# jbejjani2022/InferBiomechanics

Measured on AMD Instinct MI355X. Metric: motion-windows/sec training (+ DDIM steps/sec), higher is better.
Workload: dtype bf16; 1 GPU; transformer_denoiser_T50_D300_B256_bf16 (BASELINE.json configs[2]); per_gpu_batch=256, global_batch=256, window=50, feat=300, optimizer=rmsprop, hipgraph=True, parallelism=dp1, grad_buckets=0, overlap_comm=False, loop_stream=trainer (HipTrainer.adopt_stream, as cli/train.py)

## Files before the change

__graft_entry__.py:

```python
import os
import subprocess
import sys

ROOT = os.path.dirname(os.path.abspath(__file__))
if ROOT not in sys.path:
    sys.path.insert(0, ROOT)


def build() -> None:
    csrc = os.path.join(ROOT, "inferbiomechanics_amd", "csrc")
    jobs = str(min(8, os.cpu_count() or 1))
    subprocess.run(["make", "-C", csrc, "-j", jobs, "ARCH=gfx950"], check=True)
    from inferbiomechanics_amd import hip
    lib = hip.lib()
    missing = [s for s in hip.declared_symbols() + hip.stitch_symbols() + hip.head_symbols() + hip.sde_symbols() + hip.cfg_symbols()
               + hip.ensemble_symbols() + hip.clip_decls() + hip.standardize_decls() + hip.sched_decls() + hip.decay_decls()
               if not hasattr(lib, s)]
    if missing:
        raise RuntimeError(f"libib_hip.so does not export: {missing}")
    import inferbiomechanics_amd


def smoke() -> None:
    import argparse

    import torch

    from inferbiomechanics_amd import hip
    from inferbiomechanics_amd.loss.DiffusionLossEvaluator import DiffusionLossEvaluator
    from inferbiomechanics_amd.loss.RegressionLossEvaluator import RegressionLossEvaluator
    from inferbiomechanics_amd.models.DiffusionDenoisers import DiffusionMLP
# ... 99 lines not shown
```

inferbiomechanics_amd/csrc/ffn_chain.h:

```cpp
#pragma once
#include "wave_prims.h"
#include <utility>

#ifdef IB_AB
extern long long* g_ffn_prof;
#endif

namespace {

constexpr int FF_ROWS = 64, FF_WAVES = 8, FF_THREADS = 512, FF_D = 512, FF_CHUNK = 512, FF_MAXCHUNK = 8;
constexpr int FF_NT = 4, FF_KB = 16;
constexpr int FF_RS = FF_D * 2 + 16;
constexpr int FF_BUF = FF_ROWS * FF_RS;
constexpr int64_t FF_WELEMS = (int64_t)FF_CHUNK * FF_D;

template <int CTRL>
__device__ __forceinline__ float ff_dpp_mov(float v) {
  return __builtin_bit_cast(float, __builtin_amdgcn_update_dpp(0, __builtin_bit_cast(int, v), CTRL, 0xF, 0xF, true));
}
template <int CTRL, int ROWMASK>
__device__ __forceinline__ float ff_dpp_bcast_add(float v) {
  return v + __builtin_bit_cast(float, __builtin_amdgcn_update_dpp(0, __builtin_bit_cast(int, v), CTRL, ROWMASK, 0xF, false));
}
__device__ __forceinline__ float ff_row_sum(float a) {
// ... 91 lines not shown

__device__ __forceinline__ int ff_fresh(int v) {
  asm volatile("" : "+v"(v));
  return v;
}
__device__ __forceinline__ int ff_colb() {
  const int t = ff_fresh(threadIdx.x);
  return (t & (FF_THREADS - 64)) | 4 * ((t >> 4) & 3);
}

template <class P>
using ff_karg_t = const __attribute__((address_space(4))) P;
template <class P>
__device__ __forceinline__ ff_karg_t<P>& ff_kargs() {
  return *(ff_karg_t<P>*)__builtin_amdgcn_kernarg_segment_ptr();
}


__device__ __forceinline__ void ff_ln_rows_fwd(unsigned char* img, bool back, int nrows, int wave_s, int lane,
                                               const float (&gm)[8], const float (&bt)[8], float eps, bf16_t* yg, bf16_t* sg,
                                               float* mean_g, float* rstd_g) {
  const float invH = 1.f / (float)FF_D;
  const int c8 = lane * 8;
  constexpr int G = 2;
#pragma unroll
  for (int j0 = 0; j0 < FF_ROWS / FF_WAVES; j0 += G) {
    if (!back && wave_s + FF_WAVES * j0 >= nrows) break;
    uint4 q[G];
    float v[G][8], s1[G], sq[G];
#pragma unroll
// ... 20 lines not shown
#pragma unroll
      for (int k = 0; k < 8; ++k) hv[k] = (v[gi][k] - mean) * rstd * gm[k] + bt[k];
      const uint4 hq = ff_pack8(hv);
      if (back) *reinterpret_cast<uint4*>(img + r * FF_RS + c8 * 2) = hq;
      if (r < nrows) {
        if (yg) *reinterpret_cast<uint4*>(yg + (int64_t)r * FF_D + c8) = hq;
        if (sg) {
          *reinterpret_cast<uint4*>(sg + (int64_t)r * FF_D + c8) = q[gi];
          if (lane == 0) { mean_g[r] = mean; rstd_g[r] = rstd; }
        }
      }
    }
  }
}

template <bool FROM_IMG>
__device__ __forceinline__ void ff_ln_rows_bwd(const bf16_t* dyg, const unsigned char* dyimg, const bf16_t* sg,
                                               const float* mean_g, const float* rstd_g, const float* gamma, int nrows,
                                               int wave_s, int lane, unsigned char* zimg, bf16_t* dzg, float (&dgam)[8],
                                               float (&dbet)[8]) {
  constexpr int NJ = FF_ROWS / FF_WAVES;
  const float invH = 1.f / (float)FF_D;
  const int c8 = lane * 8;
  uint4 qd[NJ], qs[NJ];
  float2 st[NJ];
#pragma unroll
  for (int j = 0; j < NJ; ++j) {
    const int r = wave_s + FF_WAVES * j, rc = min(r, nrows - 1);
    if constexpr (FROM_IMG) qd[j] = *reinterpret_cast<const uint4*>(dyimg + r * FF_RS + c8 * 2);
    else qd[j] = *reinterpret_cast<const uint4*>(dyg + (int64_t)rc * FF_D + c8);
    qs[j] = *reinterpret_cast<const uint4*>(sg + (int64_t)rc * FF_D + c8);
    st[j] = make_float2(mean_g[rc], rstd_g[rc]);
  }
  float gm[8];
  ff_load8f(gamma + c8, gm);
#pragma unroll
  for (int k = 0; k < 8; ++k) { dgam[k] = 0.f; dbet[k] = 0.f; }
  constexpr int G = 2;
#pragma unroll
  for (int j0 = 0; j0 < NJ; j0 += G) {
    float dxh[G][8], xh[G][8], sa[G], sb[G];
#pragma unroll
    for (int gi = 0; gi < G; ++gi) {
      const bool ok = wave_s + FF_WAVES * (j0 + gi) < nrows;
      float d[8], sv[8];
      ff_unpack8(qd[j0 + gi], d);
      ff_unpack8(qs[j0 + gi], sv);
      sa[gi] = 0.f; sb[gi] = 0.f;
#pragma unroll
      for (int k = 0; k < 8; ++k) {
// ... 9 lines not shown
#pragma unroll
    for (int gi = 0; gi < G; ++gi) { sa[gi] = ff_row_sum(sa[gi]); sb[gi] = ff_row_sum(sb[gi]); }
#pragma unroll
    for (int gi = 0; gi < G; ++gi) {
      const int r = wave_s + FF_WAVES * (j0 + gi);
      const float ma = sa[gi] * invH, mb = sb[gi] * invH;
      float dz[8];
#pragma unroll
      for (int k = 0; k < 8; ++k) dz[k] = st[j0 + gi].y * (dxh[gi][k] - ma - xh[gi][k] * mb);
      const uint4 zq = ff_pack8(dz);
      *reinterpret_cast<uint4*>(zimg + r * FF_RS + c8 * 2) = zq;
      if (r < nrows) *reinterpret_cast<uint4*>(dzg + (int64_t)r * FF_D + c8) = zq;
    }
  }
}
__device__ __forceinline__ void ff_colsum_put(float* cr, int wave, int lane, const float (&dgam)[8], const float (&dbet)[8]) {
  const int c8 = lane * 8;
  float* c0 = cr + (0 * FF_WAVES + wave) * FF_D + c8;
  float* c1 = cr + (1 * FF_WAVES + wave) * FF_D + c8;
  *reinterpret_cast<float4*>(c0) = make_float4(dgam[0], dgam[1], dgam[2], dgam[3]);
  *reinterpret_cast<float4*>(c0 + 4) = make_float4(dgam[4], dgam[5], dgam[6], dgam[7]);
  *reinterpret_cast<float4*>(c1) = make_float4(dbet[0], dbet[1], dbet[2], dbet[3]);
  *reinterpret_cast<float4*>(c1 + 4) = make_float4(dbet[4], dbet[5], dbet[6], dbet[7]);
}
__device__ __forceinline__ void ff_colsum_out(const float* cr, float* partial, int q0, int tid) {
  float s0 = 0.f, s1 = 0.f;
#pragma unroll
  for (int w = 0; w < FF_WAVES; ++w) {
    s0 += cr[(0 * FF_WAVES + w) * FF_D + tid];
    s1 += cr[(1 * FF_WAVES + w) * FF_D + tid];
// ... 85 lines not shown
```

inferbiomechanics_amd/csrc/ffn_chain.hip:

```cpp
#include "ffn_chain.h"
#include "../../include/ib_hip_head.h"
#include "head_jobs.h"

#ifdef IB_AB
long long* g_ffn_prof = nullptr;
#endif
namespace {

struct FfnFwdParams {
  const bf16_t* x1;
  const bf16_t* w1p; const bf16_t* w2p;
  const float* b1; const float* b2; const float* gamma; const float* beta;
  bf16_t* f1;
  bf16_t* s2;
  bf16_t* y;
  float* mean; float* rstd;
  uint2* mask;
  const bf16_t* attn; const bf16_t* wop; const float* bo; const float* gamma1; const float* beta1;
  bf16_t* s1; bf16_t* x1out; float* mean1; float* rstd1;
  const bf16_t* wqkvp; const float* bqkv; bf16_t* qkv;
  bf16_t* attn_next; float* lse_next;
  int M, P, FF, nchunk;
  float ln_eps;
  long long* prof;
};

template <bool OUT, bool QKV, bool ATT, bool INFER = false>
__global__ __launch_bounds__(FF_THREADS) void ffn_chain_fwd_kernel(FfnFwdParams) {
  ff_karg_t<FfnFwdParams>& p = ff_kargs<FfnFwdParams>();
  static_assert(!ATT || QKV, "the attention rides behind the QKV tail");
  static_assert(!INFER || (OUT && !ATT), "the frozen-weight form: attention epilogue, no attention tail");
  __shared__ __attribute__((aligned(16))) unsigned char smem[2 * FF_BUF];
  unsigned char* imgX = smem;
  unsigned char* imgH = smem + FF_BUF;
  const int tid = threadIdx.x, lane = tid & 63, wave = tid >> 6;
  const int wave_s = __builtin_amdgcn_readfirstlane(wave);
  const int g = lane >> 4, l16 = lane & 15;
  const int r0 = blockIdx.x * p.P;
  const int nrows = min(p.P, p.M - r0);
  const int colb = wave * 16 * FF_NT + 4 * g;
  const int c8 = lane * 8;
  IB_STAMP(p.prof, 64, 0, tid == 0);
  ff_panel_in(p.x1 + (int64_t)r0 * FF_D, imgX, nrows, tid);
  if constexpr (OUT) {
    ff_panel_in(p.attn + (int64_t)r0 * FF_D, imgH, nrows, tid);
    __syncthreads();
    f32x4_t acco[4][FF_NT];
    ff_zero(acco);
    float4 bo4[FF_NT];
    auto sideo = [&](auto, int kb) {
      if (kb == FF_KB - 1) {
#pragma unroll
        for (int u = 0; u < FF_NT; ++u) bo4[u] = *reinterpret_cast<const float4*>(p.bo + colb + 16 * u);
      }
    };
    ff_gemm<FF_RING_B>(p.wop, wave_s * FF_NT, imgH, lane_now(), acco, sideo);
    float gm1[8], bt1[8];
    ff_load8f(p.gamma1 + c8, gm1);
// ... 186 lines not shown
          *reinterpret_cast<bf16x4_t*>(imgH + (16 * it + l16) * FF_RS + (colb + 16 * dt) * 2) =
              ff_pack4(o[dt][0] * inv_l[it], o[dt][1] * inv_l[it], o[dt][2] * inv_l[it], o[dt][3] * inv_l[it]);
        }
      }
      __syncthreads();
      bf16_t* ag = p.attn_next + (int64_t)r0 * FF_D;
#pragma unroll
      for (int j = 0; j < 8; ++j) ff_out_piece(imgH, ag, FF_D, nrows, ff_fresh(tid + j * FF_THREADS));
    }
#pragma unroll
    for (int j = 0; j < 8; ++j) ff_out_piece(imgX, qg + 2 * FF_CHUNK, 3 * FF_D, nrows, ff_fresh(tid + j * FF_THREADS));
    IB_STAMP(p.prof, 64, 9 + 4 * p.nchunk, tid == 0);
  }
}


struct FfnPackDesc { const bf16_t* src; int64_t ld; int transpose; int pad; bf16_t* dst; };
constexpr int FF_MAXDESC = 96;
struct FfnPackParams { FfnPackDesc d[FF_MAXDESC]; int count; };
constexpr int FF_BLOCKS_PER_DESC = 32 * FF_KB;

constexpr int FF_MAXTR = 16, FF_MAXCAST = 2;
struct FfnPackExtra { TrMultiT<FF_MAXTR> tr; CastJob cast[FF_MAXCAST]; int pack_blocks, tr_blocks, cast_blocks[FF_MAXCAST]; };

__device__ __forceinline__ void ffn_pack_body(const FfnPackParams& p, bf16_t (*tile)[32][17], int first, int stride) {
  const int lane = threadIdx.x & 63, w = threadIdx.x >> 6;
  const int total = p.count * FF_BLOCKS_PER_DESC;
  for (int blk = first; blk < total; blk += stride) {
    const FfnPackDesc& d = p.d[blk / FF_BLOCKS_PER_DESC];
    const int local = blk % FF_BLOCKS_PER_DESC;
// ... 48 lines not shown
    }
    b -= x.cast_blocks[j];
  }
}

}

#ifdef IB_AB
extern "C" int ib_debug_set_ffn_prof(void* buf) { g_ffn_prof = reinterpret_cast<long long*>(buf); return IB_OK; }
#else
extern "C" int ib_debug_set_ffn_prof(void*) { return IB_E_UNSUPPORTED; }
#endif

extern "C" int ib_ffn_chain_supported(int64_t d, int64_t ffn) {
  return (d == FF_D && ffn > 0 && ffn % FF_CHUNK == 0 && ffn / FF_CHUNK <= FF_MAXCHUNK) ? 1 : 0;
}
extern "C" size_t ib_ffn_chain_packed_elems(int64_t d, int64_t ffn) {
  return ib_ffn_chain_supported(d, ffn) ? (size_t)((4 * (ffn / FF_CHUNK) + 8) * FF_WELEMS) : 0;
}
extern "C" int ib_ffn_chain_workgroups(int64_t M, int64_t d, int64_t ffn, int* rows_per_wg) {
  int P = 0, nc = 0;
  const int n = ffn_geometry(M, d, ffn, &P, &nc);
  if (rows_per_wg) *rows_per_wg = P;
  return n;
}
extern "C" size_t ib_ffn_chain_mask_bytes(int64_t M, int64_t d, int64_t ffn) {
  int P = 0, nc = 0;
  const int n = ffn_geometry(M, d, ffn, &P, &nc);
  return (size_t)n * nc * FF_THREADS * sizeof(uint2);
}
// ... 121 lines not shown
  const bf16_t* pk = reinterpret_cast<const bf16_t*>(packed);
  p.x1 = (const bf16_t*)x1; p.w1p = pk; p.w2p = pk + (int64_t)nc * FF_WELEMS;
  p.b1 = b1; p.b2 = b2; p.gamma = gamma; p.beta = beta;
  p.f1 = (bf16_t*)f1; p.s2 = (bf16_t*)s2; p.y = (bf16_t*)y; p.mean = mean; p.rstd = rstd; p.mask = (uint2*)mask;
  p.attn = (const bf16_t*)attn; p.wop = pk + (int64_t)4 * nc * FF_WELEMS; p.bo = bo; p.gamma1 = gamma1; p.beta1 = beta1;
  p.s1 = (bf16_t*)s1; p.x1out = (bf16_t*)x1_out; p.mean1 = mean1; p.rstd1 = rstd1;
  const bool tail = qkv_next != nullptr;
  if (tail && (!out || !packed_next || !bqkv_next || !ib_al16({packed_next, bqkv_next, qkv_next}))) return IB_E_ARG;
  if (att && (!tail || !lse_next || T <= 0 || P != T || !ib_al16({attn_next}))) return IB_E_ARG;
  p.wqkvp = tail ? reinterpret_cast<const bf16_t*>(packed_next) + (int64_t)(4 * nc + 2) * FF_WELEMS : nullptr;
  p.bqkv = bqkv_next; p.qkv = (bf16_t*)qkv_next;
  p.attn_next = (bf16_t*)attn_next; p.lse_next = lse_next;
  p.M = (int)M; p.P = P; p.FF = (int)ffn; p.nchunk = nc; p.ln_eps = ln_eps;
  p.prof = IB_AB_PROF(g_ffn_prof);
  IB_PATH(IB_PATH_FFN_CHAIN);
  if (att) hipLaunchKernelGGL((ffn_chain_fwd_kernel<true, true, true>), dim3(nwg), dim3(FF_THREADS), 0, ib_s(stream), p);
  else if (tail) hipLaunchKernelGGL((ffn_chain_fwd_kernel<true, true, false>), dim3(nwg), dim3(FF_THREADS), 0, ib_s(stream), p);
  else if (out) hipLaunchKernelGGL((ffn_chain_fwd_kernel<true, false, false>), dim3(nwg), dim3(FF_THREADS), 0, ib_s(stream), p);
  else hipLaunchKernelGGL((ffn_chain_fwd_kernel<false, false, false>), dim3(nwg), dim3(FF_THREADS), 0, ib_s(stream), p);
  IB_CHECK_LAUNCH();
  return IB_OK;
}
}

extern "C" int ib_ffn_chain_fwd(const void* x1, const void* packed, const float* b1, const float* b2, const float* gamma,
                                const float* beta, void* f1, void* s2, void* y, float* mean, float* rstd, void* mask,
                                const void* attn, const float* bo, const float* gamma1, const float* beta1, void* s1,
                                void* x1_out, float* mean1, float* rstd1, const void* packed_next, const float* bqkv_next,
                                void* qkv_next, int64_t M, int64_t d, int64_t ffn, float ln_eps, ib_stream_t stream) {
  return ffn_chain_fwd_launch(x1, packed, b1, b2, gamma, beta, f1, s2, y, mean, rstd, mask, attn, bo, gamma1, beta1, s1, x1_out,
                              mean1, rstd1, packed_next, bqkv_next, qkv_next, nullptr, nullptr, 0, M, d, ffn, ln_eps, stream);
}
extern "C" int ib_ffn_chain_fwd_infer(const void* x, const void* packed, const float* b1, const float* b2, const float* gamma,
                                      const float* beta, void* y, const void* attn, const float* bo, const float* gamma1,
// ... 35 lines not shown
```

inferbiomechanics_amd/csrc/ffn_chain_bwd.hip:

```cpp
#include "ffn_chain.h"

namespace {

struct FfnBwdParams {
  const bf16_t* dy;
  const bf16_t* s2;
  const float* mean; const float* rstd; const float* gamma;
  const bf16_t* w2tp; const bf16_t* w1tp;
  const uint2* mask;
  bf16_t* ds2;
  bf16_t* dz1;
  bf16_t* dx1;
  float* partial;
  const bf16_t* s1; const float* mean1; const float* rstd1; const float* gamma1; const bf16_t* wotp;
  bf16_t* ds1;
  bf16_t* dattn;
  const bf16_t* wqkvtp; const bf16_t* dqkv_next; const bf16_t* ds1_next;
  const bf16_t* qkv; const float* lse; bf16_t* dqkv; bf16_t* dx; const bf16_t* wqkvtp_own;
  int M, P, FF, nchunk;
  long long* prof;
};

__device__ __forceinline__ void ff_qkv_dgrad(const bf16_t* addend, const bf16_t* dq, const bf16_t* wqkvtp, unsigned char* imgZ,
                                             unsigned char* imgD, int nrows, int tid, int wave_s, int l16, int colb) {
  ff_panel_in(addend, imgZ, nrows, tid);
  ff_panel_in(dq, imgD, nrows, tid, 3 * FF_D);
  __syncthreads();
  f32x4_t accd[4][FF_NT];
  ff_zero(accd);
  for (int c = 0; c < 3; ++c) {
    uint4 n0, n1, n2, n3, n4, n5, n6, n7;
    n0 = n1 = n2 = n3 = n4 = n5 = n6 = n7 = make_uint4(0u, 0u, 0u, 0u);
    const bf16_t* dqn = dq + min(c + 1, 2) * FF_CHUNK;
    auto piece = [&](int j) {
      const int idx = FF_TIDV + j * FF_THREADS;
      return *reinterpret_cast<const uint4*>(reinterpret_cast<const unsigned char*>(dqn + (int64_t)min(idx >> 6, nrows - 1) * (3 * FF_D)) + (idx & 63) * 16);
    };
    auto sided = [&](auto kbc, int) {
      constexpr int kb = decltype(kbc)::value;
      if constexpr (kb == 0) n0 = piece(0);
// ... 17 lines not shown
    }
  }
#pragma unroll
  for (int u = 0; u < FF_NT; ++u) {
#pragma unroll
    for (int mt = 0; mt < 4; ++mt) {
      bf16x4_t* slot = reinterpret_cast<bf16x4_t*>(imgZ + (16 * mt + l16) * FF_RS + (colb + 16 * u) * 2);
      const bf16x4_t av = *slot;
      *slot = ff_pack4(accd[mt][u][0] + (float)av[0], accd[mt][u][1] + (float)av[1], accd[mt][u][2] + (float)av[2],
                       accd[mt][u][3] + (float)av[3]);
    }
  }
  __syncthreads();
}

template <bool OUT, bool QKVH, bool ATT>
__global__ __launch_bounds__(FF_THREADS) void ffn_chain_bwd_kernel(FfnBwdParams) {
  ff_karg_t<FfnBwdParams>& p = ff_kargs<FfnBwdParams>();
  static_assert(!ATT || OUT, "the attention backward rides behind the out-projection's dgrad");
  __shared__ float attL[ATT ? FF_WAVES : 1][64], attD[ATT ? FF_WAVES : 1][64];
  __shared__ __attribute__((aligned(16))) unsigned char smem[2 * FF_BUF];
  unsigned char* imgZ = smem;
  unsigned char* imgD = smem + FF_BUF;
  static_assert(2 * FF_WAVES * FF_D * 4 <= FF_BUF, "dgamma / dbeta exchange must fit an image");
  const int tid = threadIdx.x, lane = tid & 63, wave = tid >> 6;
  const int wave_s = __builtin_amdgcn_readfirstlane(wave);
  const int g = lane >> 4, l16 = lane & 15;
  const int r0 = blockIdx.x * p.P;
  const int nrows = min(p.P, p.M - r0);
  IB_STAMP(p.prof, 64, 0, tid == 0);
  if constexpr (QKVH) {
    ff_qkv_dgrad(p.ds1_next + (int64_t)r0 * FF_D, p.dqkv_next + (int64_t)r0 * (3 * FF_D), p.wqkvtp, imgZ, imgD, nrows, tid,
                 wave_s, l16, ff_colb());
  }
  {
    float dgam[8], dbet[8];
    ff_ln_rows_bwd<QKVH>(p.dy + (int64_t)r0 * FF_D, imgZ, p.s2 + (int64_t)r0 * FF_D, p.mean + r0, p.rstd + r0, p.gamma, nrows,
                         wave_s, lane, imgZ, p.ds2 + (int64_t)r0 * FF_D, dgam, dbet);
    ff_colsum_put(reinterpret_cast<float*>(imgD), wave, lane, dgam, dbet);
  }
  __syncthreads();
  ff_colsum_out(reinterpret_cast<const float*>(imgD), p.partial, 0, tid);
  __syncthreads();
  IB_STAMP(p.prof, 64, 1, tid == 0);

  f32x4_t accx[4][FF_NT];
  ff_zero(accx);
  for (int c = 0; c < p.nchunk; ++c) {
    f32x4_t acca[4][FF_NT];
    ff_zero(acca);
    uint2 mk = make_uint2(0u, 0u);
    auto sideA = [&](auto, int kb) {
      if (kb == FF_KB - 1) mk = p.mask[((int64_t)blockIdx.x * p.nchunk + c) * FF_THREADS + FF_TIDV];
// ... 253 lines not shown
      for (int u = 0; u < FF_NT; ++u) {
#pragma unroll
        for (int mt = 0; mt < 4; ++mt) {
          bf16x4_t* slot = reinterpret_cast<bf16x4_t*>(imgD + (16 * mt + l16) * FF_RS + (cb + 16 * u) * 2);
          const bf16x4_t av = *slot;
          *slot = ff_pack4(accd[mt][u][0] + (float)av[0], accd[mt][u][1] + (float)av[1], accd[mt][u][2] + (float)av[2],
                           accd[mt][u][3] + (float)av[3]);
        }
      }
      __syncthreads();
      IB_STAMP(p.prof, 64, 10, tid == 0);
      ff_panel_out(imgD, p.dx + (int64_t)r0 * FF_D, nrows, tid);
      IB_STAMP(p.prof, 64, 11, tid == 0);
    }
  }
}

}

namespace {
int ffn_chain_bwd_launch(const void* dy, const void* s2, const float* mean, const float* rstd, const float* gamma,
                         const void* packed, const void* mask, void* ds2, void* dz1, void* dx1, float* partial,
                         const void* s1, const float* mean1, const float* rstd1, const float* gamma1, void* ds1,
                         void* dattn, const void* packed_next, const void* dqkv_next, const void* ds1_next,
                         const void* qkv, const float* lse, void* dqkv, void* dx, int64_t T, int64_t M, int64_t d,
                         int64_t ffn, ib_stream_t stream) {
  FfnBwdParams p{};
  int P = 0, nc = 0;
  const bool att = dqkv != nullptr;
  const int nwg = ffn_geometry(M, d, ffn, &P, &nc, att ? T : 0);
// ... 7 lines not shown
  if (att && (!out || head || !qkv || !lse || !dx || T <= 0 || P != T || !ib_al16({qkv, dqkv, dx}))) return IB_E_ARG;
  const bf16_t* pk = reinterpret_cast<const bf16_t*>(packed);
  p.dy = (const bf16_t*)dy; p.s2 = (const bf16_t*)s2; p.mean = mean; p.rstd = rstd; p.gamma = gamma;
  p.w2tp = pk + (int64_t)2 * nc * FF_WELEMS; p.w1tp = pk + (int64_t)3 * nc * FF_WELEMS;
  p.mask = (const uint2*)mask; p.ds2 = (bf16_t*)ds2; p.dz1 = (bf16_t*)dz1; p.dx1 = (bf16_t*)dx1;
  p.partial = partial;
  p.s1 = (const bf16_t*)s1; p.mean1 = mean1; p.rstd1 = rstd1; p.gamma1 = gamma1;
  p.wotp = pk + (int64_t)(4 * nc + 1) * FF_WELEMS; p.ds1 = (bf16_t*)ds1; p.dattn = (bf16_t*)dattn;
  p.wqkvtp = head ? reinterpret_cast<const bf16_t*>(packed_next) + (int64_t)(4 * nc + 5) * FF_WELEMS : nullptr;
  p.dqkv_next = (const bf16_t*)dqkv_next; p.ds1_next = (const bf16_t*)ds1_next;
  p.qkv = (const bf16_t*)qkv; p.lse = lse; p.dqkv = (bf16_t*)dqkv; p.dx = (bf16_t*)dx;
  p.wqkvtp_own = pk + (int64_t)(4 * nc + 5) * FF_WELEMS;
  p.M = (int)M; p.P = P; p.FF = (int)ffn; p.nchunk = nc;
  p.prof = IB_AB_PROF(g_ffn_prof);
  IB_PATH(IB_PATH_FFN_CHAIN);
  if (att) hipLaunchKernelGGL((ffn_chain_bwd_kernel<true, false, true>), dim3(nwg), dim3(FF_THREADS), 0, ib_s(stream), p);
  else if (head) hipLaunchKernelGGL((ffn_chain_bwd_kernel<true, true, false>), dim3(nwg), dim3(FF_THREADS), 0, ib_s(stream), p);
  else if (out) hipLaunchKernelGGL((ffn_chain_bwd_kernel<true, false, false>), dim3(nwg), dim3(FF_THREADS), 0, ib_s(stream), p);
  else hipLaunchKernelGGL((ffn_chain_bwd_kernel<false, false, false>), dim3(nwg), dim3(FF_THREADS), 0, ib_s(stream), p);
  IB_CHECK_LAUNCH();
  return IB_OK;
}
}

extern "C" int ib_ffn_chain_bwd(const void* dy, const void* s2, const float* mean, const float* rstd, const float* gamma,
                                const void* packed, const void* mask, void* ds2, void* dz1, void* dx1, float* partial,
                                const void* s1, const float* mean1, const float* rstd1, const float* gamma1, void* ds1,
                                void* dattn, const void* packed_next, const void* dqkv_next, const void* ds1_next, int64_t M,
                                int64_t d, int64_t ffn, ib_stream_t stream) {
  return ffn_chain_bwd_launch(dy, s2, mean, rstd, gamma, packed, mask, ds2, dz1, dx1, partial, s1, mean1, rstd1, gamma1, ds1,
                              dattn, packed_next, dqkv_next, ds1_next, nullptr, nullptr, nullptr, nullptr, 0, M, d, ffn, stream);
}
extern "C" int ib_ffn_chain_bwd_attn(const void* dy, const void* s2, const float* mean, const float* rstd, const float* gamma,
                                     const void* packed, const void* mask, void* ds2, void* dz1, float* partial,
// ... 8 lines not shown
```

inferbiomechanics_amd/hip.py:

```python
from __future__ import annotations

import ctypes
import os
import re
from typing import Dict, List, Optional, Sequence

import torch

_HERE = os.path.dirname(os.path.abspath(__file__))
LIB_PATH = os.environ.get("IB_HIP_LIB") or os.path.join(_HERE, "lib", "libib_hip.so")
AB_LIB_PATH = os.path.join(_HERE, "lib", "ab", "libib_hip_ab.so")
HEADER_PATH = os.path.join(os.path.dirname(_HERE), "include", "ib_hip.h")
STITCH_HEADER_PATH = os.path.join(os.path.dirname(_HERE), "include", "ib_hip_stitch.h")
HEAD_HEADER_PATH = os.path.join(os.path.dirname(_HERE), "include", "ib_hip_head.h")
SDE_HEADER_PATH = os.path.join(os.path.dirname(_HERE), "include", "ib_hip_sde.h")
CFG_HEADER_PATH = os.path.join(os.path.dirname(_HERE), "include", "ib_hip_cfg.h")
RESAMPLE_HEADER_PATH = os.path.join(os.path.dirname(_HERE), "include", "ib_hip_resample.h")
ENSEMBLE_HEADER_PATH = os.path.join(os.path.dirname(_HERE), "include", "ib_hip_ensemble.h")
CLIP_HEADER_PATH = os.path.join(os.path.dirname(_HERE), "include", "ib_hip_clip.h")
STANDARDIZE_HEADER_PATH = os.path.join(os.path.dirname(_HERE), "include", "ib_hip_standardize.h")
SCHED_HEADER_PATH = os.path.join(os.path.dirname(_HERE), "include", "ib_hip_sched.h")
DECAY_HEADER_PATH = os.path.join(os.path.dirname(_HERE), "include", "ib_hip_decay.h")

F32, BF16 = 0, 1
ACT = {"none": 0, "identity": 0, None: 0, "relu": 1, "tanh": 2, "sigmoid": 3, "silu": 4, "elu": 5}
OPT = {"sgd": 0, "adam": 1, "rmsprop": 2, "adagrad": 3, "adadelta": 4, "adamax": 5}
OPT_NUM_STATES = {"sgd": 0, "adam": 2, "rmsprop": 1, "adagrad": 1, "adadelta": 2, "adamax": 2}


class HipError(RuntimeError):
    pass


_lib = None

_c = ctypes
_vp, _i64, _i32, _f32, _sz = _c.c_void_p, _c.c_int64, _c.c_int32, _c.c_float, _c.c_size_t
# ... 49 lines not shown
_HEADERS = _TABLES + (_ENSEMBLE_SIGS, _CLIP_SIGS)
_STANDARDIZE_SIGS = _parse_header(_read_header(STANDARDIZE_HEADER_PATH))
_EVERY_HEADER = _HEADERS + (_STANDARDIZE_SIGS,)
_ALL_SIGS = {_n: _v for _t in _EVERY_HEADER for _n, _v in _t.items()}
if len(_ALL_SIGS) != sum(len(_t) for _t in _EVERY_HEADER):
    _twice = sorted(n for n in _ALL_SIGS if sum(n in _t for _t in _EVERY_HEADER) > 1)
    raise HipError(f"declared in two headers: {_twice}")
_SCHED_SIGS = _parse_header(_read_header(SCHED_HEADER_PATH))
_BOUND = {**_ALL_SIGS, **_SCHED_SIGS}
if len(_BOUND) != len(_ALL_SIGS) + len(_SCHED_SIGS):
    raise HipError(f"declared in two headers: {sorted(n for n in _SCHED_SIGS if n in _ALL_SIGS)}")
_DECAY_SIGS = _parse_header(_read_header(DECAY_HEADER_PATH))
_LOADED = {**_BOUND, **_DECAY_SIGS}
if len(_LOADED) != len(_BOUND) + len(_DECAY_SIGS):
    raise HipError(f"declared in two headers: {sorted(n for n in _DECAY_SIGS if n in _BOUND)}")
_kmax = re.search(r"^[ \t]*#[ \t]*define[ \t]+IB_STITCH_KMAX[ \t]+(\d+)[ \t]*$", _read_header(STITCH_HEADER_PATH), flags=re.M)
if _kmax is None:
    raise HipError(f"{STITCH_HEADER_PATH} does not define IB_STITCH_KMAX")
STITCH_KMAX = int(_kmax.group(1))


def declared_symbols() -> List[str]:
    return sorted(_SIGS)


def stitch_symbols() -> List[str]:
    return sorted(_STITCH_SIGS)


def head_symbols() -> List[str]:
# ... 20 lines not shown
    return sorted(_CLIP_SIGS)


def standardize_decls() -> List[str]:
    return sorted(_STANDARDIZE_SIGS)


def sched_decls() -> List[str]:
    return sorted(_SCHED_SIGS)


def decay_decls() -> List[str]:
    return sorted(_DECAY_SIGS)


def _sig(name: str):
    return _LOADED[name]


_HOST_ONLY = ("_workspace", "_supported", "_workgroups", "_packed_elems", "_partial_width", "_last_path", "_slab_count",
              "_ticket_words", "_mask_bytes", "_table_bytes")
_HOST_NAMES = ("ib_version", "ib_error_string")


def _is_launch(name: str, handed_through=("ib_event", "ib_graph")) -> bool:
    return name.startswith("ib_") and not name.startswith(tuple(handed_through)) and not name.endswith(_HOST_ONLY) \
        and name not in _HOST_NAMES


class _DryRunLib:

    def __init__(self, real):
        self._real = real
        self.calls = []
        self.ema_ranges = []
        self.args = []
# ... 215 lines not shown


def set_dry_run(on: bool):
    global _dry_run, _lib
    _dry_run = bool(on)
    _lib = None


def lib():
    global _lib
    if _lib is None:
        if not os.path.exists(LIB_PATH):
            raise HipError(f"{LIB_PATH} is missing: build it with `python -c 'import __graft_entry__ as g; g.build()'` "
                           f"or `make -C inferbiomechanics_amd/csrc` (hipcc --offload-arch=gfx950). There is no fallback path.")
        l = ctypes.CDLL(LIB_PATH)
        for name, (res, args) in _LOADED.items():
            fn = getattr(l, name)
            fn.restype = res
            fn.argtypes = args
        _lib = _DryRunLib(l) if _dry_run else l
    return _lib


def measurement_build() -> bool:
    return os.path.basename(LIB_PATH) != "libib_hip.so"


def _check(rc: int, what: str):
    if rc != 0:
        raise HipError(f"{what} failed: {lib().ib_error_string(rc).decode()} (code {rc})")

# ... 1014 lines not shown

def ffn_chain_supported(d: int, ffn: int) -> bool:
    return bool(lib().ib_ffn_chain_supported(int(d), int(ffn)))


def ffn_chain_packed_elems(d: int, ffn: int) -> int:
    return int(lib().ib_ffn_chain_packed_elems(int(d), int(ffn)))


def ffn_chain_workgroups(M: int, d: int, ffn: int, T: int = 0) -> int:
    if T:
        return int(lib().ib_ffn_chain_attn_workgroups(int(M), int(d), int(ffn), int(T)))
    return int(lib().ib_ffn_chain_workgroups(int(M), int(d), int(ffn), None))


def ffn_chain_mask_bytes(M: int, d: int, ffn: int, T: int = 0) -> int:
    if T:
        return int(lib().ib_ffn_chain_attn_mask_bytes(int(M), int(d), int(ffn), int(T)))
    return int(lib().ib_ffn_chain_mask_bytes(int(M), int(d), int(ffn)))


FFN_PACK_MAX_TRANSPOSES, FFN_PACK_MAX_CASTS = 16, 2


def ffn_chain_pack(layers, transposes=None, casts=None):
    n = len(layers)
    ffn, d = layers[0][0].shape
    for it in layers:
        w1, w2, pk = it[0], it[1], it[2]
        _mat(w1, "w1", torch.bfloat16)
# ... 1363 lines not shown
```

Baseline: 146,200 windows/s.

## Prefetch packed weight images into L2 with a grid-striped sweep in chain kernels

At the start of the fused FFN-chain forward and backward kernels, every workgroup issues a few 16-byte loads covering its own slice of the packed weight images (out-proj, W1, W2, QKV). Together these slices sweep the whole weight set once across the grid, so later reads by all workgroups should hit in cache instead of each one stalling on DRAM. The loaded values are consumed by an empty asm after the first panel load so the compiler keeps them. In exchange each workgroup holds extra vector registers for the prefetch and adds address arithmetic, and the sweep size is capped per workgroup.

```diff
diff --git a/__graft_entry__.py b/__graft_entry__.py
--- a/__graft_entry__.py
+++ b/__graft_entry__.py
@@ -15,6 +15,7 @@
     lib = hip.lib()
     missing = [s for s in hip.declared_symbols() + hip.stitch_symbols() + hip.head_symbols() + hip.sde_symbols() + hip.cfg_symbols()
                + hip.ensemble_symbols() + hip.clip_decls() + hip.standardize_decls() + hip.sched_decls() + hip.decay_decls()
+               + hip.sweep_decls()
                if not hasattr(lib, s)]
     if missing:
         raise RuntimeError(f"libib_hip.so does not export: {missing}")
diff --git a/include/ib_hip_sweep.h b/include/ib_hip_sweep.h
--- /dev/null
+++ b/include/ib_hip_sweep.h
@@ -0,0 +1,16 @@
+#ifndef IB_HIP_SWEEP_H
+#define IB_HIP_SWEEP_H
+
+#include "ib_hip.h"
+
+#ifdef __cplusplus
+extern "C" {
+#endif
+
+int ib_image_sweep_slices(int backward, int out, int qkv, int att, int64_t d, int64_t ffn, int grid, int wg,
+                          int64_t* part_bytes, int64_t* off, int64_t* len);
+
+#ifdef __cplusplus
+}
+#endif
+#endif
diff --git a/inferbiomechanics_amd/csrc/ffn_chain.h b/inferbiomechanics_amd/csrc/ffn_chain.h
--- a/inferbiomechanics_amd/csrc/ffn_chain.h
+++ b/inferbiomechanics_amd/csrc/ffn_chain.h
@@ -1,5 +1,6 @@
 #pragma once
 #include "wave_prims.h"
+#include "image_sweep.h"
 #include <utility>
 
 #ifdef IB_AB
@@ -129,6 +130,60 @@
 template <class P>
 __device__ __forceinline__ ff_karg_t<P>& ff_kargs() {
   return *(ff_karg_t<P>*)__builtin_amdgcn_kernarg_segment_ptr();
+}
+
+constexpr int FF_WBYTES = (int)(FF_WELEMS * sizeof(bf16_t));
+__host__ __device__ inline void ff_sweep_parts_fwd(bool out, bool qkv, int nchunk, int (&part)[IB_SWEEP_PARTS]) {
+  part[0] = out ? FF_WBYTES : 0;
+  part[1] = part[2] = nchunk * FF_WBYTES;
+  part[3] = qkv ? 3 * FF_WBYTES : 0;
+  part[4] = 0;
+}
+__host__ __device__ inline void ff_sweep_parts_bwd(bool out, bool qkvh, bool att, int nchunk, int (&part)[IB_SWEEP_PARTS]) {
+  part[0] = qkvh ? 3 * FF_WBYTES : 0;
+  part[1] = part[2] = nchunk * FF_WBYTES;
+  part[3] = out ? FF_WBYTES : 0;
+  part[4] = att ? 3 * FF_WBYTES : 0;
+}
+#ifdef IB_AB
+#define FF_SWEEP_TPARAM , bool FF_SWEEP_ON = true
+#else
+#define FF_SWEEP_TPARAM
+constexpr bool FF_SWEEP_ON = true;
+#endif
+struct FfSweep { u32x4_t v[IB_SWEEP_LOADS]; };
+__device__ __forceinline__ void ff_sweep_issue(const bf16_t* const (&ptr)[IB_SWEEP_PARTS], const int (&part)[IB_SWEEP_PARTS],
+                                               int tid, FfSweep& s) {
+  int off[IB_SWEEP_PARTS], len[IB_SWEEP_PARTS];
+  const int bytes = ib_sweep_slices(part, (int)gridDim.x, (int)blockIdx.x, off, len);
+  tid = ff_fresh(tid);
+#pragma unroll
+  for (int j = 0; j < IB_SWEEP_LOADS; ++j) {
+    const int u = (j * FF_THREADS + tid) * 16;
+    s.v[j] = u32x4_t{0u, 0u, 0u, 0u};
+    if (u < bytes) {
+      const unsigned char* a = nullptr;
+      int start = 0;
+#pragma unroll
+      for (int k = 0; k < IB_SWEEP_PARTS; ++k) {
+        if (u >= start && u < start + len[k]) a = reinterpret_cast<const unsigned char*>(ptr[k]) + off[k] + (u - start);
+        start += len[k];
+      }
+      s.v[j] = *reinterpret_cast<const u32x4_t*>(a);
+    }
+  }
+  __builtin_amdgcn_sched_barrier(0);
+}
+__device__ __forceinline__ void ff_sweep_drop(const FfSweep& s) {
+  static_assert(IB_SWEEP_LOADS == 3, "one operand per load");
+  asm volatile("" ::"v"(s.v[0]), "v"(s.v[1]), "v"(s.v[2]));
+}
+
+template <class P>
+__device__ __forceinline__ ff_karg_t<P>& ff_kargs_fresh() {
+  ff_karg_t<P>* q = (ff_karg_t<P>*)__builtin_amdgcn_kernarg_segment_ptr();
+  asm volatile("" : "+s"(q));
+  return *q;
 }
 
 
@@ -179,11 +234,11 @@
   }
 }
 
-template <bool FROM_IMG>
+template <bool FROM_IMG, class Requested>
 __device__ __forceinline__ void ff_ln_rows_bwd(const bf16_t* dyg, const unsigned char* dyimg, const bf16_t* sg,
                                                const float* mean_g, const float* rstd_g, const float* gamma, int nrows,
                                                int wave_s, int lane, unsigned char* zimg, bf16_t* dzg, float (&dgam)[8],
-                                               float (&dbet)[8]) {
+                                               float (&dbet)[8], Requested&& requested) {
   constexpr int NJ = FF_ROWS / FF_WAVES;
   const float invH = 1.f / (float)FF_D;
   const int c8 = lane * 8;
@@ -199,6 +254,7 @@
   }
   float gm[8];
   ff_load8f(gamma + c8, gm);
+  requested();
 #pragma unroll
   for (int k = 0; k < 8; ++k) { dgam[k] = 0.f; dbet[k] = 0.f; }
   constexpr int G = 2;
@@ -238,6 +294,13 @@
     }
   }
 }
+template <bool FROM_IMG>
+__device__ __forceinline__ void ff_ln_rows_bwd(const bf16_t* dyg, const unsigned char* dyimg, const bf16_t* sg,
+                                               const float* mean_g, const float* rstd_g, const float* gamma, int nrows,
+                                               int wave_s, int lane, unsigned char* zimg, bf16_t* dzg, float (&dgam)[8],
+                                               float (&dbet)[8]) {
+  ff_ln_rows_bwd<FROM_IMG>(dyg, dyimg, sg, mean_g, rstd_g, gamma, nrows, wave_s, lane, zimg, dzg, dgam, dbet, [] {});
+}
 __device__ __forceinline__ void ff_colsum_put(float* cr, int wave, int lane, const float (&dgam)[8], const float (&dbet)[8]) {
   const int c8 = lane * 8;
   float* c0 = cr + (0 * FF_WAVES + wave) * FF_D + c8;
diff --git a/inferbiomechanics_amd/csrc/ffn_chain.hip b/inferbiomechanics_amd/csrc/ffn_chain.hip
--- a/inferbiomechanics_amd/csrc/ffn_chain.hip
+++ b/inferbiomechanics_amd/csrc/ffn_chain.hip
@@ -1,5 +1,6 @@
 #include "ffn_chain.h"
 #include "../../include/ib_hip_head.h"
+#include "../../include/ib_hip_sweep.h"
 #include "head_jobs.h"
 
 #ifdef IB_AB
@@ -25,9 +26,10 @@
   long long* prof;
 };
 
-template <bool OUT, bool QKV, bool ATT, bool INFER = false>
+template <bool OUT, bool QKV, bool ATT, bool INFER = false FF_SWEEP_TPARAM>
 __global__ __launch_bounds__(FF_THREADS) void ffn_chain_fwd_kernel(FfnFwdParams) {
   ff_karg_t<FfnFwdParams>& p = ff_kargs<FfnFwdParams>();
+  constexpr bool SWEEP = FF_SWEEP_ON && !INFER;
   static_assert(!ATT || QKV, "the attention rides behind the QKV tail");
   static_assert(!INFER || (OUT && !ATT), "the frozen-weight form: attention epilogue, no attention tail");
   __shared__ __attribute__((aligned(16))) unsigned char smem[2 * FF_BUF];
@@ -41,7 +43,16 @@
   const int colb = wave * 16 * FF_NT + 4 * g;
   const int c8 = lane * 8;
   IB_STAMP(p.prof, 64, 0, tid == 0);
+  [[maybe_unused]] FfSweep sweep;
+  if constexpr (SWEEP) {
+    int part[IB_SWEEP_PARTS];
+    ff_karg_t<FfnFwdParams>& ps = ff_kargs_fresh<FfnFwdParams>();
+    ff_sweep_parts_fwd(OUT, QKV, ps.nchunk, part);
+    const bf16_t* const parts[IB_SWEEP_PARTS] = {OUT ? ps.wop : nullptr, ps.w1p, ps.w2p, QKV ? ps.wqkvp : nullptr, nullptr};
+    ff_sweep_issue(parts, part, tid, sweep);
+  }
   ff_panel_in(p.x1 + (int64_t)r0 * FF_D, imgX, nrows, tid);
+  if constexpr (SWEEP) ff_sweep_drop(sweep);
   if constexpr (OUT) {
     ff_panel_in(p.attn + (int64_t)r0 * FF_D, imgH, nrows, tid);
     __syncthreads();
@@ -258,6 +269,18 @@
   }
 }
 
+template <bool OUT, bool QKV, bool ATT>
+void ffn_chain_fwd_go(int nwg, ib_stream_t stream, const FfnFwdParams& p) {
+#ifdef IB_AB
+  static const bool no_sweep = ib_ab_set("IB_NO_IMAGE_SWEEP");
+  if (no_sweep) {
+    hipLaunchKernelGGL((ffn_chain_fwd_kernel<OUT, QKV, ATT, false, false>), dim3(nwg), dim3(FF_THREADS), 0, ib_s(stream), p);
+    return;
+  }
+#endif
+  hipLaunchKernelGGL((ffn_chain_fwd_kernel<OUT, QKV, ATT>), dim3(nwg), dim3(FF_THREADS), 0, ib_s(stream), p);
+}
+
 
 struct FfnPackDesc { const bf16_t* src; int64_t ld; int transpose; int pad; bf16_t* dst; };
 constexpr int FF_MAXDESC = 96;
@@ -336,6 +359,20 @@
 
 extern "C" int ib_ffn_chain_supported(int64_t d, int64_t ffn) {
   return (d == FF_D && ffn > 0 && ffn % FF_CHUNK == 0 && ffn / FF_CHUNK <= FF_MAXCHUNK) ? 1 : 0;
+}
+extern "C" int ib_image_sweep_slices(int backward, int out, int qkv, int att, int64_t d, int64_t ffn, int grid, int wg,
+                                     int64_t* part_bytes, int64_t* off, int64_t* len) {
+  if (!ib_ffn_chain_supported(d, ffn)) return IB_E_UNSUPPORTED;
+  if (!part_bytes || !off || !len || grid < 1 || wg < 0 || wg >= grid) return IB_E_ARG;
+  const bool o = out != 0, q = qkv != 0, a = att != 0;
+  if (backward ? ((q || a) && !o) || (q && a) : (a && !q) || (q && !o)) return IB_E_ARG;
+  int part[IB_SWEEP_PARTS], po[IB_SWEEP_PARTS], pl[IB_SWEEP_PARTS];
+  const int nc = (int)(ffn / FF_CHUNK);
+  if (backward) ff_sweep_parts_bwd(o, q, a, nc, part);
+  else ff_sweep_parts_fwd(o, q, nc, part);
+  const int bytes = ib_sweep_slices(part, grid, wg, po, pl);
+  for (int k = 0; k < IB_SWEEP_PARTS; ++k) { part_bytes[k] = part[k]; off[k] = po[k]; len[k] = pl[k]; }
+  return bytes;
 }
 extern "C" size_t ib_ffn_chain_packed_elems(int64_t d, int64_t ffn) {
   return ib_ffn_chain_supported(d, ffn) ? (size_t)((4 * (ffn / FF_CHUNK) + 8) * FF_WELEMS) : 0;
@@ -487,10 +524,10 @@
   p.M = (int)M; p.P = P; p.FF = (int)ffn; p.nchunk = nc; p.ln_eps = ln_eps;
   p.prof = IB_AB_PROF(g_ffn_prof);
   IB_PATH(IB_PATH_FFN_CHAIN);
-  if (att) hipLaunchKernelGGL((ffn_chain_fwd_kernel<true, true, true>), dim3(nwg), dim3(FF_THREADS), 0, ib_s(stream), p);
-  else if (tail) hipLaunchKernelGGL((ffn_chain_fwd_kernel<true, true, false>), dim3(nwg), dim3(FF_THREADS), 0, ib_s(stream), p);
-  else if (out) hipLaunchKernelGGL((ffn_chain_fwd_kernel<true, false, false>), dim3(nwg), dim3(FF_THREADS), 0, ib_s(stream), p);
-  else hipLaunchKernelGGL((ffn_chain_fwd_kernel<false, false, false>), dim3(nwg), dim3(FF_THREADS), 0, ib_s(stream), p);
+  if (att) ffn_chain_fwd_go<true, true, true>(nwg, stream, p);
+  else if (tail) ffn_chain_fwd_go<true, true, false>(nwg, stream, p);
+  else if (out) ffn_chain_fwd_go<true, false, false>(nwg, stream, p);
+  else ffn_chain_fwd_go<false, false, false>(nwg, stream, p);
   IB_CHECK_LAUNCH();
   return IB_OK;
 }
diff --git a/inferbiomechanics_amd/csrc/ffn_chain_bwd.hip b/inferbiomechanics_amd/csrc/ffn_chain_bwd.hip
--- a/inferbiomechanics_amd/csrc/ffn_chain_bwd.hip
+++ b/inferbiomechanics_amd/csrc/ffn_chain_bwd.hip
@@ -21,9 +21,12 @@
   long long* prof;
 };
 
+template <class Landed>
 __device__ __forceinline__ void ff_qkv_dgrad(const bf16_t* addend, const bf16_t* dq, const bf16_t* wqkvtp, unsigned char* imgZ,
-                                             unsigned char* imgD, int nrows, int tid, int wave_s, int l16, int colb) {
+                                             unsigned char* imgD, int nrows, int tid, int wave_s, int l16, int colb,
+                                             Landed&& landed) {
   ff_panel_in(addend, imgZ, nrows, tid);
+  landed();
   ff_panel_in(dq, imgD, nrows, tid, 3 * FF_D);
   __syncthreads();
   f32x4_t accd[4][FF_NT];
@@ -71,9 +74,10 @@
   __syncthreads();
 }
 
-template <bool OUT, bool QKVH, bool ATT>
+template <bool OUT, bool QKVH, bool ATT FF_SWEEP_TPARAM>
 __global__ __launch_bounds__(FF_THREADS) void ffn_chain_bwd_kernel(FfnBwdParams) {
   ff_karg_t<FfnBwdParams>& p = ff_kargs<FfnBwdParams>();
+  constexpr bool SWEEP = FF_SWEEP_ON;
   static_assert(!ATT || OUT, "the attention backward rides behind the out-projection's dgrad");
   __shared__ float attL[ATT ? FF_WAVES : 1][64], attD[ATT ? FF_WAVES : 1][64];
   __shared__ __attribute__((aligned(16))) unsigned char smem[2 * FF_BUF];
@@ -86,14 +90,24 @@
   const int r0 = blockIdx.x * p.P;
   const int nrows = min(p.P, p.M - r0);
   IB_STAMP(p.prof, 64, 0, tid == 0);
+  [[maybe_unused]] FfSweep sweep;
+  if constexpr (SWEEP) {
+    int part[IB_SWEEP_PARTS];
+    ff_karg_t<FfnBwdParams>& ps = ff_kargs_fresh<FfnBwdParams>();
+    ff_sweep_parts_bwd(OUT, QKVH, ATT, ps.nchunk, part);
+    const bf16_t* const parts[IB_SWEEP_PARTS] = {QKVH ? ps.wqkvtp : nullptr, ps.w2tp, ps.w1tp, OUT ? ps.wotp : nullptr,
+                                                 ATT ? ps.wqkvtp_own : nullptr};
+    ff_sweep_issue(parts, part, tid, sweep);
+  }
   if constexpr (QKVH) {
     ff_qkv_dgrad(p.ds1_next + (int64_t)r0 * FF_D, p.dqkv_next + (int64_t)r0 * (3 * FF_D), p.wqkvtp, imgZ, imgD, nrows, tid,
-                 wave_s, l16, ff_colb());
+                 wave_s, l16, ff_colb(), [&] { if constexpr (SWEEP) ff_sweep_drop(sweep); });
   }
   {
     float dgam[8], dbet[8];
     ff_ln_rows_bwd<QKVH>(p.dy + (int64_t)r0 * FF_D, imgZ, p.s2 + (int64_t)r0 * FF_D, p.mean + r0, p.rstd + r0, p.gamma, nrows,
-                         wave_s, lane, imgZ, p.ds2 + (int64_t)r0 * FF_D, dgam, dbet);
+                         wave_s, lane, imgZ, p.ds2 + (int64_t)r0 * FF_D, dgam, dbet,
+                         [&] { if constexpr (SWEEP && !QKVH) ff_sweep_drop(sweep); });
     ff_colsum_put(reinterpret_cast<float*>(imgD), wave, lane, dgam, dbet);
   }
   __syncthreads();
@@ -377,6 +391,18 @@
       IB_STAMP(p.prof, 64, 11, tid == 0);
     }
   }
+}
+
+template <bool OUT, bool QKVH, bool ATT>
+void ffn_chain_bwd_go(int nwg, ib_stream_t stream, const FfnBwdParams& p) {
+#ifdef IB_AB
+  static const bool no_sweep = ib_ab_set("IB_NO_IMAGE_SWEEP");
+  if (no_sweep) {
+    hipLaunchKernelGGL((ffn_chain_bwd_kernel<OUT, QKVH, ATT, false>), dim3(nwg), dim3(FF_THREADS), 0, ib_s(stream), p);
+    return;
+  }
+#endif
+  hipLaunchKernelGGL((ffn_chain_bwd_kernel<OUT, QKVH, ATT>), dim3(nwg), dim3(FF_THREADS), 0, ib_s(stream), p);
 }
 
 }
@@ -414,10 +440,10 @@
   p.M = (int)M; p.P = P; p.FF = (int)ffn; p.nchunk = nc;
   p.prof = IB_AB_PROF(g_ffn_prof);
   IB_PATH(IB_PATH_FFN_CHAIN);
-  if (att) hipLaunchKernelGGL((ffn_chain_bwd_kernel<true, false, true>), dim3(nwg), dim3(FF_THREADS), 0, ib_s(stream), p);
-  else if (head) hipLaunchKernelGGL((ffn_chain_bwd_kernel<true, true, false>), dim3(nwg), dim3(FF_THREADS), 0, ib_s(stream), p);
-  else if (out) hipLaunchKernelGGL((ffn_chain_bwd_kernel<true, false, false>), dim3(nwg), dim3(FF_THREADS), 0, ib_s(stream), p);
-  else hipLaunchKernelGGL((ffn_chain_bwd_kernel<false, false, false>), dim3(nwg), dim3(FF_THREADS), 0, ib_s(stream), p);
+  if (att) ffn_chain_bwd_go<true, false, true>(nwg, stream, p);
+  else if (head) ffn_chain_bwd_go<true, true, false>(nwg, stream, p);
+  else if (out) ffn_chain_bwd_go<true, false, false>(nwg, stream, p);
+  else ffn_chain_bwd_go<false, false, false>(nwg, stream, p);
   IB_CHECK_LAUNCH();
   return IB_OK;
 }
diff --git a/inferbiomechanics_amd/csrc/image_sweep.h b/inferbiomechanics_amd/csrc/image_sweep.h
--- /dev/null
+++ b/inferbiomechanics_amd/csrc/image_sweep.h
@@ -0,0 +1,29 @@
+#pragma once
+#include <stdint.h>
+
+constexpr int IB_SWEEP_PARTS = 5;
+constexpr int IB_SWEEP_LOADS = 3;
+constexpr int IB_SWEEP_CAP = IB_SWEEP_LOADS * 512 * 16;
+
+__host__ __device__ inline int ib_sweep_slices(const int (&part)[IB_SWEEP_PARTS], int grid, int wg, int (&off)[IB_SWEEP_PARTS],
+                                               int (&len)[IB_SWEEP_PARTS]) {
+  int total = 0;
+#pragma unroll
+  for (int k = 0; k < IB_SWEEP_PARTS; ++k) total += part[k];
+  int q = ((total + grid - 1) / grid + 15) & ~15;
+  if (q > IB_SWEEP_CAP) q = IB_SWEEP_CAP;
+  const int64_t lo64 = (int64_t)wg * q;
+  const int lo = lo64 < total ? (int)lo64 : total;
+  const int hi = lo64 + q < total ? (int)(lo64 + q) : total;
+  int base = 0, bytes = 0;
+#pragma unroll
+  for (int k = 0; k < IB_SWEEP_PARTS; ++k) {
+    const int a = lo > base ? lo : base;
+    const int b = hi < base + part[k] ? hi : base + part[k];
+    len[k] = b > a ? b - a : 0;
+    off[k] = b > a ? a - base : 0;
+    bytes += len[k];
+    base += part[k];
+  }
+  return bytes;
+}
diff --git a/inferbiomechanics_amd/hip.py b/inferbiomechanics_amd/hip.py
--- a/inferbiomechanics_amd/hip.py
+++ b/inferbiomechanics_amd/hip.py
@@ -21,6 +21,7 @@
 STANDARDIZE_HEADER_PATH = os.path.join(os.path.dirname(_HERE), "include", "ib_hip_standardize.h")
 SCHED_HEADER_PATH = os.path.join(os.path.dirname(_HERE), "include", "ib_hip_sched.h")
 DECAY_HEADER_PATH = os.path.join(os.path.dirname(_HERE), "include", "ib_hip_decay.h")
+SWEEP_HEADER_PATH = os.path.join(os.path.dirname(_HERE), "include", "ib_hip_sweep.h")
 
 F32, BF16 = 0, 1
 ACT = {"none": 0, "identity": 0, None: 0, "relu": 1, "tanh": 2, "sigmoid": 3, "silu": 4, "elu": 5}
@@ -100,6 +101,10 @@
 _LOADED = {**_BOUND, **_DECAY_SIGS}
 if len(_LOADED) != len(_BOUND) + len(_DECAY_SIGS):
     raise HipError(f"declared in two headers: {sorted(n for n in _DECAY_SIGS if n in _BOUND)}")
+_SWEEP_SIGS = _parse_header(_read_header(SWEEP_HEADER_PATH))
+_ENTRIES = {**_LOADED, **_SWEEP_SIGS}
+if len(_ENTRIES) != len(_LOADED) + len(_SWEEP_SIGS):
+    raise HipError(f"declared in two headers: {sorted(n for n in _SWEEP_SIGS if n in _LOADED)}")
 _kmax = re.search(r"^[ \t]*#[ \t]*define[ \t]+IB_STITCH_KMAX[ \t]+(\d+)[ \t]*$", _read_header(STITCH_HEADER_PATH), flags=re.M)
 if _kmax is None:
     raise HipError(f"{STITCH_HEADER_PATH} does not define IB_STITCH_KMAX")
@@ -150,12 +155,16 @@
     return sorted(_DECAY_SIGS)
 
 
+def sweep_decls() -> List[str]:
+    return sorted(_SWEEP_SIGS)
+
+
 def _sig(name: str):
-    return _LOADED[name]
+    return _ENTRIES[name]
 
 
 _HOST_ONLY = ("_workspace", "_supported", "_workgroups", "_packed_elems", "_partial_width", "_last_path", "_slab_count",
-              "_ticket_words", "_mask_bytes", "_table_bytes")
+              "_ticket_words", "_mask_bytes", "_table_bytes", "_sweep_slices")
 _HOST_NAMES = ("ib_version", "ib_error_string")
 
 
@@ -401,7 +410,7 @@
             raise HipError(f"{LIB_PATH} is missing: build it with `python -c 'import __graft_entry__ as g; g.build()'` "
                            f"or `make -C inferbiomechanics_amd/csrc` (hipcc --offload-arch=gfx950). There is no fallback path.")
         l = ctypes.CDLL(LIB_PATH)
-        for name, (res, args) in _LOADED.items():
+        for name, (res, args) in _ENTRIES.items():
             fn = getattr(l, name)
             fn.restype = res
             fn.argtypes = args
@@ -1446,6 +1455,14 @@
     return int(lib().ib_ffn_chain_workgroups(int(M), int(d), int(ffn), None))
 
 
+def image_sweep_slices(backward: bool, out: bool, qkv: bool, att: bool, d: int, ffn: int, grid: int, wg: int):
+    arr = [(ctypes.c_int64 * 5)() for _ in range(3)]
+    rc = int(lib().ib_image_sweep_slices(int(backward), int(out), int(qkv), int(att), int(d), int(ffn), int(grid), int(wg), *arr))
+    if rc < 0:
+        _check(rc, "ib_image_sweep_slices")
+    return rc, list(zip(*(list(a) for a in arr)))
+
+
 def ffn_chain_mask_bytes(M: int, d: int, ffn: int, T: int = 0) -> int:
     if T:
         return int(lib().ib_ffn_chain_attn_mask_bytes(int(M), int(d), int(ffn), int(T)))
```

New measurement: 159,300 windows/s (median of 6 runs). +9.0%, better.
